# pauxy-qmc/pauxy

Hardware: AMD Instinct MI355X
Metric: walker_steps_per_sec (higher is better)
Workload: dtype f64

## Files before the change

### pauxy_amd/csrc/k_fused.hip

```cpp
#include <cstdlib>
#include <type_traits>

#include "mfma_gemm_wg.h"

#define PF_D 3
#ifndef PF_NW
#define PF_NW 8
#endif
#define PF_NT (64 * PF_NW)
#ifndef PF_LW
#define PF_LW PF_NW
#endif
#define PF_FPW (16 / PF_LW)

#ifdef AFQ_TUNING
#define PF_UNLESS(bits) if (!(a.dbg & (bits)))
#define PF_TUNE(...) __VA_ARGS__
#define PF_STAGE(i) stage_stamp(i)
#define PF_BND(n, i) bnd_stamp(n, i)
#else
#define PF_UNLESS(bits)
#define PF_TUNE(...)
#define PF_STAGE(i)
#define PF_BND(n, i)
#endif

struct PropFusedArgs {
    int M, na, nb, nt, order;
    int t4;
    int dbg;
    unsigned long long *ts;
    int vhs_upper;
    int same_b;
    int b_real;
    int rem4;
    int hyb;
    int symcols;
    int closed_try;
    int contig;
    const cplx *BH1;
    const cplx *vhs;
    cplx *phi;
    const int *alive;
    const void *zero16;
    unsigned long long *n_closed;
};

__device__ inline d2_t lds_read_c(unsigned addr) { return lds_read_b128(addr); }

template <int OFF> __device__ inline d2_t lds_read_off(unsigned addr) {
    d2_t v;
    asm volatile("ds_read_b128 %0, %1 offset:%2" : "=v"(v) : "v"(addr), "n"(OFF));
    return v;
}
__device__ __attribute__((always_inline)) inline d2_t lds_read_frag(unsigned base, int idx) {
    switch (idx) {
    case 0: return lds_read_off<0>(base);
    case 1: return lds_read_off<1024>(base);
    case 2: return lds_read_off<2048>(base);
    case 3: return lds_read_off<3072>(base);
    case 4: return lds_read_off<4096>(base);
    case 5: return lds_read_off<5120>(base);
    case 6: return lds_read_off<6144>(base);
    default: return lds_read_off<7168>(base);
    }
}

template <int OFF> __device__ inline double lds_read_re_off(unsigned addr) {
    double v;
    asm volatile("ds_read_b64 %0, %1 offset:%2" : "=v"(v) : "v"(addr), "n"(OFF));
    return v;
}
__device__ __attribute__((always_inline)) inline double lds_read_frag_re(unsigned base, int idx) {
    switch (idx) {
    case 0: return lds_read_re_off<0>(base);
    case 1: return lds_read_re_off<1024>(base);
    case 2: return lds_read_re_off<2048>(base);
    case 3: return lds_read_re_off<3072>(base);
    case 4: return lds_read_re_off<4096>(base);
    case 5: return lds_read_re_off<5120>(base);
    case 6: return lds_read_re_off<6144>(base);
    default: return lds_read_re_off<7168>(base);
    }
}

__device__ inline void lds_barrier() {
    asm volatile("s_waitcnt lgkmcnt(0)" ::: "memory");
    __builtin_amdgcn_s_barrier();
    asm volatile("" ::: "memory");
}

template <bool NARROW, int FULL>
__global__ __launch_bounds__(PF_NT) void prop_fused_kernel(PropFusedArgs a) {
    extern __shared__ __align__(16) unsigned char smem[];
    const int w = blockIdx.x;
    if (!a.alive[w]) return;
    const int tid = threadIdx.x, lane = tid & 63, wave = __builtin_amdgcn_readfirstlane(tid >> 6);
    const int lr = lane & 15, lk = lane >> 4;
    const int M = a.M, nt = a.nt;
    const int NCH = (M + 7) >> 3;
    const int nrt = (M + 15) >> 4;
    unsigned char *Tf = smem;
    unsigned char *ring = smem + (size_t)NCH * 8192;
    const unsigned tf_l = lds_addr(Tf), ring_l = lds_addr(ring);
    cplx *phi = a.phi + (long)w * M * nt;
    const cplx *vhs = a.vhs + (long)w * M * M;

    PF_TUNE(auto stage_stamp = [&](int i) {
        if (a.ts && w == 0 && wave == 0) {
            unsigned long long t;
            asm volatile("s_memtime %0\n\ts_waitcnt lgkmcnt(0)" : "=s"(t));
            if (lane == 0) a.ts[128 + i] = t;
        }
    };
    auto bnd_stamp = [&](int n, int i) {
        if (a.ts && w == 0 && (wave & 3) == 0 && (n == 3 || n == 4)) {
            unsigned long long t;
            asm volatile("s_memtime %0\n\ts_waitcnt lgkmcnt(0)" : "=s"(t));
            if (lane == 0) a.ts[144 + (wave >> 2) * 8 + (n == 4 ? 4 : 0) + i] = t;
        }
    };)
    PF_STAGE(0);
    const int nob = a.same_b ? 1 : 2;
    const int nphase = 2 * nob + a.order;
    const int G = nphase * NCH;
    const long MM = (long)M * M;
    int gi = 0, gi_phase = 0, gi_c = 0, gi_slot = 0;
    const void *nsrc[PF_FPW];
    bool prepared = false;
    const bool refills = wave >= PF_NW - PF_LW;
    const int lw = wave - (PF_NW - PF_LW);
    const int p_row0 = (lw >> 1) * 16 + lr;
    const int p_kl = 2 * lk + (lw & 1);
    auto prepare = [&]() __attribute__((always_inline)) {
        if (!refills) { prepared = true; return; }
        PF_TUNE(if ((a.dbg & 1024) && gi > 2) { prepared = true; return; })
        const bool in_v = gi_phase >= nob && gi_phase < nob + a.order;
        const int spin = gi_phase < nob ? gi_phase : gi_phase - nob - a.order;
        const cplx *A = in_v ? vhs : a.BH1 + (spin == 1 ? MM : 0L);
        const bool sym_phase = a.vhs_upper && in_v;
        const bool live = gi < G;
        const int k = gi_c * 8 + p_kl;
#pragma unroll
        for (int t = 0; t < PF_FPW; ++t) {
            const int row = p_row0 + t * (PF_LW / 2) * 16;
            const int off = (sym_phase && k < row) ? k * M + row : row * M + k;
            nsrc[t] = (live && row < M && k < M) ? (const void *)(A + off) : a.zero16;
            asm volatile("" : "+v"(nsrc[t]));
        }
        ++gi;
        const bool wrap = gi_c + 1 == NCH;
        gi_c = wrap ? 0 : gi_c + 1;
        gi_phase += wrap ? 1 : 0;
        prepared = true;
    };
    auto issueA = [&]() __attribute__((always_inline)) {
        if (!refills) return;
        if (!prepared) prepare();
        unsigned char *dst = ring + (size_t)gi_slot * 16384;
        PF_TUNE(if (a.dbg & 512) { for (int t = 0; t < PF_FPW; ++t) asm volatile("" ::"v"(nsrc[t]), "s"(dst)); } else)
#pragma unroll
        for (int t = 0; t < PF_FPW; ++t) glds16(nsrc[t], dst + (lw + t * PF_LW) * 1024);
        if (++gi_slot == PF_D) gi_slot = 0;
        prepared = false;
    };
    issueA(); issueA();
    prepare();
    bool closed = false;
    if (a.closed_try) {
        bool same = true;
        for (int p = tid >> 5; p < M; p += PF_NT / 32) {
            const int c = tid & 31;
            if (c < a.na) {
                const cplx x = phi[p * nt + c], y = phi[p * nt + a.na + c];
                same = same && __double_as_longlong(x.x) == __double_as_longlong(y.x) &&
                       __double_as_longlong(x.y) == __double_as_longlong(y.y);
            }
        }
        closed = __builtin_amdgcn_readfirstlane(__syncthreads_and(same ? 1 : 0)) != 0;
        if (closed && tid == 0) atomicAdd(a.n_closed, 1ULL);
    }
    const bool relayout = closed && a.contig;
    const int contig = relayout ? 0 : a.contig, hyb = relayout ? 0 : a.hyb;
    const int sym_n = (a.symcols && !relayout) ? a.na : 0;
    auto wcol = [&](const int c) -> int {
        if (!sym_n) return c;
        if (c < 16) return c;
        if (c < 32) return sym_n + (c - 16);
        if (c < 40) return 16 + (c - 32);
        if (c < 48) return sym_n + 16 + (c - 40);
        const int e = c - 48, extra = sym_n - 24;
        return e < extra ? 24 + e : sym_n + 24 + (e - extra);
    };

    PF_UNLESS((32 | 128))
    for (int e = tid; e < NCH * 512; e += PF_NT) {
        const int j = e & 15, kk = (e >> 4) & 3, pb = (e >> 6) & 1, slot = (e >> 7) & 3, ch = e >> 9;
        const int p = ch * 8 + 2 * kk + pb, sp = contig ? 0 : slot >> 1, col = (contig ? slot : slot & 1) * 16 + j;
        const int ns_ = contig ? nt : sp ? a.nb : a.na, off_ = sp ? a.na : 0;
        const bool ok = p < M && col < ns_;
        const cplx v = phi[ok ? p * nt + off_ + wcol(col) : 0];
        ((d2_t *)Tf)[e] = ok ? (d2_t){v.x, v.y} : (d2_t){0.0, 0.0};
    }
    __syncthreads();

    auto t_ok = [&](int ti, int r) -> bool { return 2 * ti + (r >> 1) < NCH; };
    const unsigned t_lane = (unsigned)((lk & 1) * 1024 + ((lk >> 1) * 16 + lr) * 16);
    auto t_addr = [&](int ti, int r, int cs) -> unsigned {
        unsigned base = t_lane;
        asm volatile("" : "+v"(base));
        return base + (unsigned)(((2 * ti * 4 + cs) * 2) * 1024) + (unsigned)((r >> 1) * 8192 + (r & 1) * 512);
    };

    PF_STAGE(1);
    int ring_slot = 0;
    auto next_chunk = [&]() __attribute__((always_inline)) -> unsigned {
        PF_UNLESS(18)
        asm volatile("s_waitcnt vmcnt(%0)" ::"n"((PF_D - 2) * PF_FPW) : "memory");
        PF_UNLESS(1)
        __builtin_amdgcn_s_barrier();
        PF_UNLESS(2)
        issueA();
        const unsigned sl = ring_l + ring_slot * 16384;
        if (++ring_slot == PF_D) ring_slot = 0;
        return sl;
    };
    auto next_chunk_sync = [&]() __attribute__((always_inline)) -> unsigned {
        asm volatile("s_waitcnt vmcnt(%0)" ::"n"((PF_D - 2) * PF_FPW) : "memory");
        __builtin_amdgcn_s_barrier();
        const unsigned sl = ring_l + ring_slot * 16384;
        ring_slot = ring_slot + 1 == PF_D ? 0 : ring_slot + 1;
        return sl;
    };

    auto one_body = [&](auto nsl_tag, int slot0, bool to_global, auto real_tag, const int rt) __attribute__((always_inline)) {
        constexpr int NSL = decltype(nsl_tag)::value;
        constexpr bool BR = decltype(real_tag)::value;
        constexpr int SS = (NARROW && FULL) ? 2 : 1;
        d4_t P1[NSL], P2[NSL], P3[NSL];
        bool cv[NSL];
#pragma unroll
        for (int j = 0; j < NSL; ++j) {
            P1[j] = (d4_t){0, 0, 0, 0}; P2[j] = (d4_t){0, 0, 0, 0}; P3[j] = (d4_t){0, 0, 0, 0};
            const int cs = slot0 + j * SS;
            cv[j] = rt < nrt && (cs & 1) < ((((cs >> 1) ? a.nb : a.na) + 15) >> 4);
        }
        auto load_frags = [&](unsigned sl, int c, d2_t (&av)[2], d2_t (&bv)[NSL][2]) {
            const unsigned abase = sl + rt * 2048 + lane * 16;
            const unsigned bbase = tf_l + (c * 4 + slot0) * 2048 + lane * 16;
#pragma unroll
            for (int ss = 0; ss < 2; ++ss) {
                if (BR) av[ss][0] = lds_read_frag_re(abase, ss);
                else av[ss] = lds_read_frag(abase, ss);
#pragma unroll
                for (int j = 0; j < NSL; ++j) bv[j][ss] = lds_read_frag(bbase, j * SS * 2 + ss);
            }
        };
        auto mfmas = [&](d2_t (&av)[2], d2_t (&bv)[NSL][2]) {
            __builtin_amdgcn_sched_barrier(0);
            PF_UNLESS(64)
#pragma unroll
            for (int ss = 0; ss < 2; ++ss)
#pragma unroll
                for (int j = 0; j < NSL; ++j)
                    if (FULL || cv[j]) {
                        if (BR) {
                            P1[j] = mfma16(av[ss][0], bv[j][ss][0], P1[j]);
                            P2[j] = mfma16(av[ss][0], bv[j][ss][1], P2[j]);
                        } else {
                            P1[j] = mfma16(av[ss][0], bv[j][ss][0], P1[j]);
                            P2[j] = mfma16(av[ss][1], bv[j][ss][1], P2[j]);
                            P3[j] = mfma16(av[ss][0] + av[ss][1], bv[j][ss][0] + bv[j][ss][1], P3[j]);
                        }
                    }
            __builtin_amdgcn_sched_barrier(0);
            if (!prepared) prepare();
            asm volatile("s_waitcnt lgkmcnt(0)" ::: "memory");
        };
#if PF_NW == 8
        if (FULL) {
            constexpr int NR = 1 + NSL;
            constexpr int RPG = NSL > 1 ? (NR + NSL - 2) / (NSL > 1 ? NSL - 1 : 1) : NR;
            d2_t a0, a1, b0[NSL], b1[NSL];
            auto half = [&](d2_t &ax, d2_t (&bx)[NSL], d2_t &ay, d2_t (&by)[NSL], const unsigned abase, const unsigned bbase,
                            const int ys, const bool fetch, const bool refill) __attribute__((always_inline)) {
                __builtin_amdgcn_sched_barrier(0);
#pragma unroll
                for (int j = 0; j < NSL; ++j) {
                    if (BR) {
                        P1[j] = mfma16(ax[0], bx[j][0], P1[j]);
                        P2[j] = mfma16(ax[0], bx[j][1], P2[j]);
                    } else {
                        P1[j] = mfma16(ax[0], bx[j][0], P1[j]);
                        P2[j] = mfma16(ax[1], bx[j][1], P2[j]);
                        P3[j] = mfma16(ax[0] + ax[1], bx[j][0] + bx[j][1], P3[j]);
                    }
                    __builtin_amdgcn_sched_barrier(0);
                    if (j == 0 && refill) issueA();
                    if (j == 0 && !refill && !prepared) prepare();
                    if (fetch && (j < NSL - 1 || NSL == 1)) {
#pragma unroll
                        for (int q = 0; q < RPG; ++q) {
                            const int r = j * RPG + q;
                            if (r < NR) {
                                if (r == 0) {
                                    if (BR) ay[0] = lds_read_frag_re(abase, ys);
                                    else ay = lds_read_frag(abase, ys);
                                }
                                else by[r - 1] = lds_read_frag(bbase, (r - 1) * SS * 2 + ys);
                            }
                        }
                    }
                    __builtin_amdgcn_sched_barrier(0);
                }
                asm volatile("s_waitcnt lgkmcnt(0)" ::: "memory");
            };
            unsigned sl = next_chunk_sync();
            {
                const unsigned abase = sl + rt * 2048 + lane * 16, bbase = tf_l + slot0 * 2048 + lane * 16;
                if (BR) a0[0] = lds_read_frag_re(abase, 0);
                else a0 = lds_read_frag(abase, 0);
#pragma unroll
                for (int j = 0; j < NSL; ++j) b0[j] = lds_read_frag(bbase, j * SS * 2);
                __builtin_amdgcn_sched_barrier(0);
                issueA();
                asm volatile("s_waitcnt lgkmcnt(0)" ::: "memory");
            }
            for (int c = 0; c < NCH; ++c) {
                const bool more = c + 1 < NCH;
                half(a0, b0, a1, b1, sl + rt * 2048 + lane * 16, tf_l + (c * 4 + slot0) * 2048 + lane * 16, 1, true, false);
                if (more) sl = next_chunk_sync();
                half(a1, b1, a0, b0, sl + rt * 2048 + lane * 16, tf_l + ((c + 1) * 4 + slot0) * 2048 + lane * 16, 0, more, more);
            }
        } else
#endif
        {
#if PF_NW == 16
        d2_t avA[2], bvA[NSL][2];
        for (int c = 0; c < NCH; ++c) {
            load_frags(next_chunk(), c, avA, bvA);
            asm volatile("s_waitcnt lgkmcnt(0)" ::: "memory");
            mfmas(avA, bvA);
        }
#else
        d2_t avA[2], bvA[NSL][2], avB[2], bvB[NSL][2];
        load_frags(next_chunk(), 0, avA, bvA);
        asm volatile("s_waitcnt lgkmcnt(0)" ::: "memory");
        for (int c = 0; c < NCH; c += 2) {
            if (c + 1 < NCH) load_frags(next_chunk(), c + 1, avB, bvB);
            mfmas(avA, bvA);
            if (c + 1 < NCH) {
                if (c + 2 < NCH) load_frags(next_chunk(), c + 2, avA, bvA);
                mfmas(avB, bvB);
            }
        }
#endif
        }
        if (!to_global) __builtin_amdgcn_s_barrier();
        int lk_e = lk, lr_e = lr;
        asm volatile("" : "+v"(lk_e), "+v"(lr_e));
#pragma unroll
        for (int j = 0; j < NSL; ++j)
            if (cv[j]) {
                const int cs = slot0 + j * SS, sp = contig ? 0 : cs >> 1;
                const int ns_ = contig ? nt : sp ? a.nb : a.na, off_ = sp ? a.na : 0;
#pragma unroll
                for (int r = 0; r < 4; ++r) {
                    const double re = BR ? P1[j][r] : P1[j][r] - P2[j][r];
                    const double im = BR ? P2[j][r] : P3[j][r] - P1[j][r] - P2[j][r];
                    if (to_global) {
                        const int row = rt * 16 + lk_e + 4 * r, col = (contig ? cs : cs & 1) * 16 + lr_e;
                        PF_UNLESS(256)
                        if (row < M && col < ns_) phi[(long)row * nt + off_ + wcol(col)] = cmake(re, im);
                    } else if (t_ok(rt, r)) {
                        *(d2_t *)(Tf + t_addr(rt, r, cs)) = (d2_t){re, im};
                    }
                }
            }
    };
    auto one_body_col = [&](bool to_global, auto real_tag, auto rem_tag) __attribute__((always_inline)) {
        constexpr bool BR = decltype(real_tag)::value;
        constexpr bool REM = decltype(rem_tag)::value;
        constexpr int NI = 3;
        constexpr int NG = NI + (REM ? 1 : 0), NR = NI + 1 + (REM ? 1 : 0), RPG = (NR + NG - 2) / (NG - 1);
        const int c0 = wave & 3, r0 = (wave >> 2) * 3;
        const unsigned rem_t = (unsigned)((((12 * 4 + c0) * 2 + ((lane >> 4) & 1)) * 1024) + (((lane >> 5) * 16) + (lane & 15)) * 16);
        const unsigned rem_a = (unsigned)(6 * 2048 + ((lane >> 4) * 16 + (lane & 3)) * 16);
        d4_t P1[NI], P2[NI], P3[NI];
#pragma unroll
        for (int i = 0; i < NI; ++i) { P1[i] = (d4_t){0, 0, 0, 0}; P2[i] = (d4_t){0, 0, 0, 0}; P3[i] = (d4_t){0, 0, 0, 0}; }
        double Q1 = 0.0, Q2 = 0.0, Q3 = 0.0;
        d2_t a0[NI], a1[NI], b0, b1, q0 = (d2_t){0.0, 0.0}, q1 = (d2_t){0.0, 0.0};
        auto half = [&](d2_t (&ax)[NI], d2_t &bx, d2_t &qx, d2_t (&ay)[NI], d2_t &by, d2_t &qy, const unsigned abase,
                        const unsigned bbase, const unsigned qbase, const int ys, const bool fetch, const bool refill)
            __attribute__((always_inline)) {
            __builtin_amdgcn_sched_barrier(0);
#pragma unroll
            for (int gt = 0; gt < NG; ++gt) {
                if (REM && gt == 0) {
                    if (BR) {
                        Q1 = __builtin_amdgcn_mfma_f64_4x4x4f64(qx[0], bx[0], Q1, 0, 0, 0);
                        Q2 = __builtin_amdgcn_mfma_f64_4x4x4f64(qx[0], bx[1], Q2, 0, 0, 0);
                    } else {
                        Q1 = __builtin_amdgcn_mfma_f64_4x4x4f64(qx[0], bx[0], Q1, 0, 0, 0);
                        Q2 = __builtin_amdgcn_mfma_f64_4x4x4f64(qx[1], bx[1], Q2, 0, 0, 0);
                        Q3 = __builtin_amdgcn_mfma_f64_4x4x4f64(qx[0] + qx[1], bx[0] + bx[1], Q3, 0, 0, 0);
                    }
                } else {
                    const int i = REM ? gt - 1 : gt;
                    if (BR) {
                        P1[i] = mfma16(ax[i][0], bx[0], P1[i]);
                        P2[i] = mfma16(ax[i][0], bx[1], P2[i]);
                    } else {
                        P1[i] = mfma16(ax[i][0], bx[0], P1[i]);
                        P2[i] = mfma16(ax[i][1], bx[1], P2[i]);
                        P3[i] = mfma16(ax[i][0] + ax[i][1], bx[0] + bx[1], P3[i]);
                    }
                }
                __builtin_amdgcn_sched_barrier(0);
                if (gt == 0 && refill) issueA();
                if (gt == 0 && !refill && !prepared) prepare();
                if (fetch && gt < NG - 1) {
#pragma unroll
                    for (int q = 0; q < RPG; ++q) {
                        const int r = gt * RPG + q;
                        if (r < NR) {
                            if (r < NI) {
                                if (BR) ay[r][0] = lds_read_frag_re(abase, r * 2 + ys);
                                else ay[r] = lds_read_frag(abase, r * 2 + ys);
                            } else if (r == NI) {
                                by = lds_read_frag(bbase, ys);
                            } else {
                                if (BR) qy[0] = lds_read_frag_re(qbase, ys);
                                else qy = lds_read_frag(qbase, ys);
                            }
                        }
                    }
                }
                __builtin_amdgcn_sched_barrier(0);
            }
            asm volatile("s_waitcnt lgkmcnt(0)" ::: "memory");
        };
        unsigned sl = next_chunk_sync();
        {
            const unsigned abase = sl + r0 * 2048 + lane * 16, bbase = tf_l + c0 * 2048 + lane * 16;
#pragma unroll
            for (int i = 0; i < NI; ++i) {
                if (BR) a0[i][0] = lds_read_frag_re(abase, i * 2);
                else a0[i] = lds_read_frag(abase, i * 2);
            }
            b0 = lds_read_frag(bbase, 0);
            if (REM) {
                if (BR) q0[0] = lds_read_frag_re(sl + rem_a, 0);
                else q0 = lds_read_frag(sl + rem_a, 0);
            }
            __builtin_amdgcn_sched_barrier(0);
            issueA();
            asm volatile("s_waitcnt lgkmcnt(0)" ::: "memory");
        }
        for (int c = 0; c < NCH; ++c) {
            const bool more = c + 1 < NCH;
            half(a0, b0, q0, a1, b1, q1, sl + r0 * 2048 + lane * 16, tf_l + (c * 4 + c0) * 2048 + lane * 16, sl + rem_a, 1, true, false);
            if (more) sl = next_chunk_sync();
            half(a1, b1, q1, a0, b0, q0, sl + r0 * 2048 + lane * 16, tf_l + ((c + 1) * 4 + c0) * 2048 + lane * 16, sl + rem_a, 0, more, more);
        }
        int lk_e = lk, lr_e = lr, ln_e = lane;
        asm volatile("" : "+v"(lk_e), "+v"(lr_e), "+v"(ln_e));
        const int sp = contig ? 0 : c0 >> 1, ns_ = contig ? nt : sp ? a.nb : a.na, off_ = sp ? a.na : 0;
        const int cb = (contig ? c0 : c0 & 1) * 16;
#pragma unroll
        for (int i = 0; i < NI; ++i)
#pragma unroll
            for (int r = 0; r < 4; ++r) {
                const double re = BR ? P1[i][r] : P1[i][r] - P2[i][r];
                const double im = BR ? P2[i][r] : P3[i][r] - P1[i][r] - P2[i][r];
                if (to_global) {
                    const int row = (r0 + i) * 16 + lk_e + 4 * r, col = cb + lr_e;
                    if (row < M && col < ns_) phi[(long)row * nt + off_ + wcol(col)] = cmake(re, im);
                } else if (t_ok(r0 + i, r)) {
                    *(d2_t *)(Tf + t_addr(r0 + i, r, c0)) = (d2_t){re, im};
                }
            }
        if (!to_global) __builtin_amdgcn_s_barrier();
        if (REM) {
            const double re = BR ? Q1 : Q1 - Q2, im = BR ? Q2 : Q3 - Q1 - Q2;
// ... 164 lines not shown
                        }
                        __builtin_amdgcn_sched_barrier(0);
                        if (gt == 0 && refill) issueA();
                        if (gt == 0 && !refill && !prepared) prepare();
                        if (fetch && (gt < NG - 1 || NG == 1)) {
#pragma unroll
                            for (int q = 0; q < RPG; ++q) {
                                const int r = gt * RPG + q;
                                if (r < NR) {
                                    if (r < NI) ay[r] = lds_read_frag(abase, r * 2 + ys);
                                    else if (r < NI + NJ) by[r - NI] = lds_read_frag(bbase, (r - NI) * 2 + ys);
                                    else qy = lds_read_frag(qbase, ys);
                                }
                            }
                        }
                        __builtin_amdgcn_sched_barrier(0);
                    }
                    asm volatile("s_waitcnt lgkmcnt(0)" ::: "memory");
                };
                unsigned sl = next_chunk_sync();
                if (n == 4) PF_BND(4, 0);
                {
                    const unsigned abase = sl + r0 * 2048 + lane * 16, bbase = tf_l + c0 * 2048 + lane * 16;
#pragma unroll
                    for (int i = 0; i < NI; ++i) a0[i] = lds_read_frag(abase, i * 2);
#pragma unroll
                    for (int j = 0; j < NJ; ++j) b0[j] = lds_read_frag(bbase, j * 2);
                    if (REM) q0 = lds_read_frag(sl + rem_a, 0);
                    __builtin_amdgcn_sched_barrier(0);
                    issueA();
                    asm volatile("s_waitcnt lgkmcnt(0)" ::: "memory");
                }
                if (n == 4) PF_BND(4, 1);
                for (int c = 0; c < NCH; ++c) {
                    const bool more = c + 1 < NCH;
                    PF_TUNE(unsigned long long t0, t1, t2, t3; asm volatile("s_memtime %0" : "=s"(t0));)
                    half(a0, b0, q0, a1, b1, q1, sl + r0 * 2048 + lane * 16, tf_l + (c * 4 + c0) * 2048 + lane * 16, sl + rem_a, 1, true, false);
                    PF_TUNE(asm volatile("s_memtime %0" : "=s"(t1));)
                    if (more) sl = next_chunk_sync();
                    PF_TUNE(asm volatile("s_memtime %0" : "=s"(t2));)
                    half(a1, b1, q1, a0, b0, q0, sl + r0 * 2048 + lane * 16, tf_l + ((c + 1) * 4 + c0) * 2048 + lane * 16, sl + rem_a, 0, more, more);
                    PF_TUNE(asm volatile("s_memtime %0\n\ts_waitcnt lgkmcnt(0)" : "=s"(t3));
                            if (a.ts && w == 0 && n == 3 && (wave & 3) == 0 && lane == 0) {
                                unsigned long long *o = a.ts + ((wave >> 2) * 16 + c) * 4;
                                o[0] = t0; o[1] = t1; o[2] = t2; o[3] = t3;
                            }
                            if (a.ts && w == 0 && n == 3 && lane == 0) {
                                unsigned long long *o = a.ts + 256 + (wave * 16 + c) * 4;
                                o[0] = t0; o[1] = t1; o[2] = t2; o[3] = t3;
                            })
                }
            } else
#endif
            {
#if PF_NW == 16
            d2_t avA[NI][2], bvA[NJ][2];
            for (int c = 0; c < NCH; ++c) {
                load_frags(next_chunk(), c, avA, bvA);
                asm volatile("s_waitcnt lgkmcnt(0)" ::: "memory");
                mfmas(avA, bvA);
            }
#else
            d2_t avA[NI][2], bvA[NJ][2], avB[NI][2], bvB[NJ][2];
            if (STAG) {
                auto half = [&](d2_t (&ax)[NI][2], d2_t (&bx)[NJ][2], d2_t (&ay)[NI][2], d2_t (&by)[NJ][2], const int c)
                    __attribute__((always_inline)) {
                    unsigned sl = 0;
                    if (c + 1 < NCH) sl = next_chunk();
                    __builtin_amdgcn_sched_barrier(0);
                    mfma_ss(ax, bx, 1);
                    __builtin_amdgcn_sched_barrier(0);
                    if (!prepared) prepare();
                    if (c + 1 < NCH) {
                        load_frags(sl, c + 1, ay, by);
                        asm volatile("s_waitcnt lgkmcnt(0)" ::: "memory");
                        __builtin_amdgcn_sched_barrier(0);
                        mfma_ss(ay, by, 0);
                        __builtin_amdgcn_sched_barrier(0);
                    }
                };
                load_frags(next_chunk(), 0, avA, bvA);
                asm volatile("s_waitcnt lgkmcnt(0)" ::: "memory");
                __builtin_amdgcn_sched_barrier(0);
                mfma_ss(avA, bvA, 0);
                __builtin_amdgcn_sched_barrier(0);
                for (int c = 0; c < NCH; c += 2) {
                    half(avA, bvA, avB, bvB, c);
                    if (c + 1 < NCH) half(avB, bvB, avA, bvA, c + 1);
                }
            } else {
                load_frags(next_chunk(), 0, avA, bvA);
                asm volatile("s_waitcnt lgkmcnt(0)" ::: "memory");
                for (int c = 0; c < NCH; c += 2) {
                    if (c + 1 < NCH) load_frags(next_chunk(), c + 1, avB, bvB);
                    mfmas(avA, bvA);
                    if (c + 1 < NCH) {
                        if (c + 2 < NCH) load_frags(next_chunk(), c + 2, avA, bvA);
                        mfmas(avB, bvB);
                    }
                }
            }
#endif
            }
            if (n == 3) PF_BND(3, 0);
            const bool store_first = PF_NW == 8 && FULL != 0 && 2 * (r0 + NI) <= NCH - 1;
            if (!store_first) __builtin_amdgcn_s_barrier();
            if (n == 3) PF_BND(3, 1);
            const bool last = n == a.order;
#pragma unroll
            for (int i = 0; i < NI; ++i)
#pragma unroll
                for (int j = 0; j < NJ; ++j)
                    if (FULL || (cv[j] && rv[i])) {
#pragma unroll
                        for (int r = 0; r < 4; ++r) {
                            const double re = (P1[i][j][r] - P2[i][j][r]) * inv_n;
                            const double im = (P3[i][j][r] - P1[i][j][r] - P2[i][j][r]) * inv_n;
                            SR[i][j][r] += re; SI[i][j][r] += im;
                            if (!last && t_ok(r0 + i, r)) *(d2_t *)(Tf + t_addr(r0 + i, r, c0 + j)) = (d2_t){re, im};
                        }
                    }
            if (last) {
#pragma unroll
                for (int i = 0; i < NI; ++i)
#pragma unroll
                    for (int j = 0; j < NJ; ++j)
                        if (FULL || (cv[j] && rv[i])) {
#pragma unroll
                            for (int r = 0; r < 4; ++r)
                                if (t_ok(r0 + i, r))
                                    *(d2_t *)(Tf + t_addr(r0 + i, r, c0 + j)) = (d2_t){SR[i][j][r], SI[i][j][r]};
                        }
            }
            if (store_first) __builtin_amdgcn_s_barrier();
            if (REM) {
                const double re = (Q1 - Q2) * inv_n, im = (Q3 - Q1 - Q2) * inv_n;
                RR += re; RI += im;
                *(d2_t *)(Tf + rem_t) = last ? (d2_t){RR, RI} : (d2_t){re, im};
            }
            if (n == 3) PF_BND(3, 2);
            asm volatile("s_waitcnt lgkmcnt(0)" ::: "memory");
            if (n == 3) PF_BND(3, 3);
            PF_STAGE(2 + n);
        }
    };

    auto taylor_h = [&](auto hf_tag, auto rem_tag, auto nu_tag, const int r0, const int cf, const int cu, const int cr)
        __attribute__((always_inline)) {
        constexpr bool HF = decltype(hf_tag)::value;
        constexpr bool HR = decltype(rem_tag)::value;
        constexpr int NU = decltype(nu_tag)::value;
        constexpr int NI = 2, NRU = HR ? 2 : 0;
        static_assert(FULL == 7, "hybrid tiling: the full wide deal");
        const unsigned u_rd = (unsigned)((lane >> 4) * 256 + (lane & 3) * 16);
        const int ui = lane >> 4, ub = (lane >> 2) & 3;
        const unsigned u_wr = (unsigned)((ub >> 1) * 8192 + (ui & 1) * 1024 + ((2 * (ub & 1) + (ui >> 1)) * 16 + (lane & 3)) * 16);
        auto u_addr = [&](int ti, int u) -> unsigned {
            unsigned base = u_wr;
            asm volatile("" : "+v"(base));
            return base + (unsigned)((2 * ti * 4 + cu) * 2048 + u * 64);
        };
        const unsigned rem_a = (unsigned)(6 * 2048 + ((lane >> 4) * 16 + (lane & 3)) * 16);
        auto rem_t = [&](int t) -> unsigned {
            return (unsigned)((((12 * 4 + cr + t) * 2 + ((lane >> 4) & 1)) * 1024) + (((lane >> 5) * 16) + (lane & 15)) * 16);
        };
        d4_t SR[NI], SI[NI];
        double UR[NI][NU], UI[NI][NU], RR[2] = {0.0, 0.0}, RI[2] = {0.0, 0.0};
#pragma unroll
        for (int i = 0; i < NI; ++i) {
#pragma unroll
            for (int r = 0; r < 4; ++r) {
                d2_t v = (d2_t){0.0, 0.0};
                if (HF) v = *(const d2_t *)(Tf + t_addr(r0 + i, r, cf));
                SR[i][r] = v[0]; SI[i][r] = v[1];
            }
#pragma unroll
            for (int u = 0; u < NU; ++u) { const d2_t v = *(const d2_t *)(Tf + u_addr(r0 + i, u)); UR[i][u] = v[0]; UI[i][u] = v[1]; }
        }
        if (HR) {
#pragma unroll
            for (int t = 0; t < 2; ++t) { const d2_t v = *(const d2_t *)(Tf + rem_t(t)); RR[t] = v[0]; RI[t] = v[1]; }
        }
        struct Frag { d2_t a[NI]; d2_t bf; d2_t bu[NU]; d2_t q; d2_t br[2]; };
        constexpr int NG = NI * NU + NRU + (HF ? NI : 0);
        constexpr int NR = NI + NU + (HF ? 1 : 0) + (HR ? 3 : 0);
        constexpr int NGAP = HF ? NG - 1 : NG - 3;
        constexpr int RPG = (NR + NGAP - 1) / NGAP;
        for (int n = 1; n <= a.order; ++n) {
            double inv_n = 1.0 / n;
            asm volatile("" : "+v"(inv_n));
            d4_t P1[NI], P2[NI], P3[NI];
            double U1[NI][NU], U2[NI][NU], U3[NI][NU], Q1[2] = {0.0, 0.0}, Q2[2] = {0.0, 0.0}, Q3[2] = {0.0, 0.0};
#pragma unroll
            for (int i = 0; i < NI; ++i) {
                P1[i] = (d4_t){0, 0, 0, 0}; P2[i] = (d4_t){0, 0, 0, 0}; P3[i] = (d4_t){0, 0, 0, 0};
#pragma unroll
                for (int u = 0; u < NU; ++u) { U1[i][u] = 0.0; U2[i][u] = 0.0; U3[i][u] = 0.0; }
            }
            auto read_one = [&](Frag &f, const int r, const unsigned sl, const int c, const int ys) __attribute__((always_inline)) {
                const unsigned abase = sl + r0 * 2048 + lane * 16;
                if (r < NI) { f.a[r] = lds_read_frag(abase, r * 2 + ys); return; }
                if (r < NI + NU) {
                    const int u = r - NI;
                    const unsigned ubase = tf_l + (c * 4 + cu) * 2048 + u_rd + ys * 1024;
                    f.bu[u] = u == 0 ? lds_read_off<0>(ubase) : u == 1 ? lds_read_off<64>(ubase) : lds_read_off<128>(ubase);
                    return;
                }
                int k = r - NI - NU;
                if (HF) {
                    if (k == 0) { f.bf = lds_read_frag(tf_l + (c * 4 + cf) * 2048 + lane * 16, ys); return; }
                    --k;
                }
                if (HR) {
                    if (k == 0) f.q = lds_read_frag(sl + rem_a, ys);
                    else f.br[k - 1] = lds_read_frag(tf_l + (c * 4 + cr + k - 1) * 2048 + lane * 16, ys);
                }
            };
            auto half = [&](Frag &x, Frag &y, const unsigned sl, const int c, const int ys, const bool fetch, const bool refill)
                __attribute__((always_inline)) {
                __builtin_amdgcn_sched_barrier(0);
#pragma unroll
                for (int g = 0; g < NG; ++g) {
                    if (g < NI * NU) {
                        const int i = g / NU, u = g % NU;
                        U1[i][u] = __builtin_amdgcn_mfma_f64_4x4x4f64(x.a[i][0], x.bu[u][0], U1[i][u], 0, 0, 0);
                        U2[i][u] = __builtin_amdgcn_mfma_f64_4x4x4f64(x.a[i][1], x.bu[u][1], U2[i][u], 0, 0, 0);
                        U3[i][u] = __builtin_amdgcn_mfma_f64_4x4x4f64(x.a[i][0] + x.a[i][1], x.bu[u][0] + x.bu[u][1], U3[i][u], 0, 0, 0);
                    } else if (g < NI * NU + NRU) {
                        const int t = g - NI * NU;
                        Q1[t] = __builtin_amdgcn_mfma_f64_4x4x4f64(x.q[0], x.br[t][0], Q1[t], 0, 0, 0);
                        Q2[t] = __builtin_amdgcn_mfma_f64_4x4x4f64(x.q[1], x.br[t][1], Q2[t], 0, 0, 0);
                        Q3[t] = __builtin_amdgcn_mfma_f64_4x4x4f64(x.q[0] + x.q[1], x.br[t][0] + x.br[t][1], Q3[t], 0, 0, 0);
                    } else {
                        const int i = g - NI * NU - NRU;
                        P1[i] = mfma16(x.a[i][0], x.bf[0], P1[i]);
                        P2[i] = mfma16(x.a[i][1], x.bf[1], P2[i]);
                        P3[i] = mfma16(x.a[i][0] + x.a[i][1], x.bf[0] + x.bf[1], P3[i]);
                    }
                    __builtin_amdgcn_sched_barrier(0);
                    if (g == 0 && refill) issueA();
                    if (g == 0 && !refill && !prepared) prepare();
                    if (fetch && g < NGAP) {
#pragma unroll
                        for (int q = 0; q < RPG; ++q)
                            if (g * RPG + q < NR) read_one(y, g * RPG + q, sl, c, ys);
                    }
                    __builtin_amdgcn_sched_barrier(0);
                }
                asm volatile("s_waitcnt lgkmcnt(0)" ::: "memory");
            };
            Frag f0, f1;
            f0.q = (d2_t){0.0, 0.0}; f1.q = (d2_t){0.0, 0.0};
            unsigned sl = next_chunk_sync();
#pragma unroll
            for (int r = 0; r < NR; ++r) read_one(f0, r, sl, 0, 0);
            __builtin_amdgcn_sched_barrier(0);
            issueA();
            asm volatile("s_waitcnt lgkmcnt(0)" ::: "memory");
            for (int c = 0; c < NCH; ++c) {
                const bool more = c + 1 < NCH;
                PF_TUNE(unsigned long long t0, t1, t2, t3; asm volatile("s_memtime %0" : "=s"(t0));)
                half(f0, f1, sl, c, 1, true, false);
                PF_TUNE(asm volatile("s_memtime %0" : "=s"(t1));)
                if (more) sl = next_chunk_sync();
                PF_TUNE(asm volatile("s_memtime %0" : "=s"(t2));)
                half(f1, f0, sl, c + 1, 0, more, more);
                PF_TUNE(asm volatile("s_memtime %0\n\ts_waitcnt lgkmcnt(0)" : "=s"(t3));
                        if (a.ts && w == 0 && n == 3 && lane == 0) {
                            unsigned long long *o = a.ts + 256 + (wave * 16 + c) * 4;
                            o[0] = t0; o[1] = t1; o[2] = t2; o[3] = t3;
                        })
            }
            const bool last = n == a.order;
#pragma unroll
            for (int i = 0; i < NI; ++i) {
                if (HF) {
#pragma unroll
                    for (int r = 0; r < 4; ++r) {
                        const double re = (P1[i][r] - P2[i][r]) * inv_n, im = (P3[i][r] - P1[i][r] - P2[i][r]) * inv_n;
                        SR[i][r] += re; SI[i][r] += im;
                        *(d2_t *)(Tf + t_addr(r0 + i, r, cf)) = last ? (d2_t){SR[i][r], SI[i][r]} : (d2_t){re, im};
                    }
                }
#pragma unroll
                for (int u = 0; u < NU; ++u) {
                    const double re = (U1[i][u] - U2[i][u]) * inv_n, im = (U3[i][u] - U1[i][u] - U2[i][u]) * inv_n;
                    UR[i][u] += re; UI[i][u] += im;
                    *(d2_t *)(Tf + u_addr(r0 + i, u)) = last ? (d2_t){UR[i][u], UI[i][u]} : (d2_t){re, im};
                }
            }
            __builtin_amdgcn_s_barrier();
            if (HR) {
#pragma unroll
                for (int t = 0; t < 2; ++t) {
                    const double re = (Q1[t] - Q2[t]) * inv_n, im = (Q3[t] - Q1[t] - Q2[t]) * inv_n;
                    RR[t] += re; RI[t] += im;
                    *(d2_t *)(Tf + rem_t(t)) = last ? (d2_t){RR[t], RI[t]} : (d2_t){re, im};
                }
            }
            asm volatile("s_waitcnt lgkmcnt(0)" ::: "memory");
        }
    };

#ifdef AFQ_TUNING
#include "k_fused_t4.inc"
#endif
    auto mirror_spin = [&]() __attribute__((always_inline)) {
        lds_barrier();
        for (int e = tid; e < NCH * 256; e += PF_NT) {
            const int ch = e >> 8, i = e & 255;
            ((d2_t *)Tf)[ch * 512 + 256 + i] = ((const d2_t *)Tf)[ch * 512 + i];
        }
        asm volatile("s_waitcnt lgkmcnt(0)" ::: "memory");
    };
#if PF_NW == 16
    {
        using I1 = std::integral_constant<int, 1>;
        using I2 = std::integral_constant<int, 2>;
        const int g = wave >> 2;
        if (g & 1) taylor(I2{}, I1{}, std::true_type{}, 2 * g, wave & 3, g == 3 ? 1 : 2, std::false_type{});
        else taylor(I2{}, I1{}, std::false_type{}, 2 * g, wave & 3, 2, std::false_type{});
    }
#else
    PF_TUNE(if (a.t4) taylor4(); else)
    if (NARROW && FULL) {
        using I1 = std::integral_constant<int, 1>;
        using I2 = std::integral_constant<int, 2>;
        if (closed) {
            taylor(I1{}, I1{}, std::false_type{}, wave < 6 ? wave : wave - 6, 0, 1, std::false_type{});
            mirror_spin();
        }
        else if (wave < 4) taylor(I2{}, I1{}, std::false_type{}, 2 * (wave & 1), 2 * (wave >> 1), 2, std::false_type{});
        else taylor(I1{}, I1{}, std::false_type{}, 4 + (wave & 1), 2 * ((wave - 4) >> 1), 1, std::false_type{});
    }
    else if (NARROW) {
        using I1 = std::integral_constant<int, 1>;
        using I2 = std::integral_constant<int, 2>;
        if (wave < 4) taylor(I2{}, I1{}, std::false_type{}, 2 * (wave & 1), 2 * (wave >> 1), 2, std::false_type{});
        else if (nrt <= 6) taylor(I2{}, I1{}, std::true_type{}, 4 + (wave & 1), 2 * ((wave - 4) >> 1), 1, std::false_type{});
        else taylor(I2{}, I1{}, std::true_type{}, (wave & 1) ? 6 : 4, 2 * ((wave - 4) >> 1), (wave & 1) ? 1 : 2, std::false_type{});
    }
    else if (FULL == 7 && contig) {
        if constexpr (FULL == 7) {
            using I1 = std::integral_constant<int, 1>;
            using I2 = std::integral_constant<int, 2>;
            auto deal = [&](auto nu) __attribute__((always_inline)) {
                if (wave == 0 || wave == 2) taylor(I2{}, I2{}, std::false_type{}, wave, 0, 2, std::false_type{});
                else if (wave == 1 || wave == 3) taylor_h(std::true_type{}, std::false_type{}, nu, wave - 1, 2, 3, 0);
                else if (wave == 4 || wave == 6) taylor(I1{}, I1{}, std::true_type{}, 4, (wave - 4) >> 1, 1, std::true_type{});
                else if (wave == 5) taylor(I1{}, I2{}, std::true_type{}, 5, 0, 1, std::false_type{});
                else taylor_h(std::true_type{}, std::true_type{}, nu, 4, 2, 3, 2);
            };
            if (hyb == 2) deal(I2{});
            else deal(I1{});
        }
    }
    else if (FULL == 7 && hyb) {
        if constexpr (FULL == 7) {
            using I1 = std::integral_constant<int, 1>;
            using I2 = std::integral_constant<int, 2>;
            using I3 = std::integral_constant<int, 3>;
            auto deal = [&](auto nu) __attribute__((always_inline)) {
                if (wave < 4) taylor_h(std::true_type{}, std::false_type{}, nu, 2 * (wave >> 1), 2 * (wave & 1), 2 * (wave & 1) + 1, 0);
                else if (wave < 6) taylor(I2{}, I1{}, std::true_type{}, 4, 2 * (wave - 4), 2, std::false_type{});
                else taylor_h(std::false_type{}, std::true_type{}, nu, 4, 0, 2 * (wave - 6) + 1, 2 * (wave - 6));
            };
            if (hyb == 3) deal(I3{});
            else if (hyb == 2) deal(I2{});
            else deal(I1{});
        }
    }
    else if (FULL >= 5 && closed) {
        using I1 = std::integral_constant<int, 1>;
        using I2 = std::integral_constant<int, 2>;
        const int cs = wave & 1;
        if (wave < 4) taylor(I2{}, I1{}, std::false_type{}, 2 * (wave >> 1), cs, 2, std::false_type{});
        else if constexpr (FULL == 7) {
            if (a.rem4) {
                if (wave < 6) taylor(I1{}, I1{}, std::true_type{}, 4, cs, 1, std::true_type{});
                else taylor(I1{}, I1{}, std::true_type{}, 5, cs, 1, std::false_type{});
            } else {
                if (wave < 6) taylor(I2{}, I1{}, std::true_type{}, 4, cs, 2, std::false_type{});
                else taylor(I1{}, I1{}, std::true_type{}, 6, cs, 1, std::false_type{});
            }
        }
        else taylor(I1{}, I1{}, std::true_type{}, (FULL == 6 && wave >= 6) ? 5 : 4, cs, 1, std::false_type{});
        mirror_spin();
    }
    else if (wave < 4) taylor(std::integral_constant<int, 2>{}, std::integral_constant<int, 2>{}, std::false_type{}, 2 * (wave >> 1), 2 * (wave & 1), 2, std::false_type{});
    else if constexpr (FULL == 7) {
        if (a.rem4) taylor(std::integral_constant<int, 2>{}, std::integral_constant<int, 1>{}, std::true_type{}, 4, wave - 4, 2, std::true_type{});
        else taylor(std::integral_constant<int, 3>{}, std::integral_constant<int, 1>{}, std::true_type{}, 4, wave - 4, 3, std::false_type{});
    }
    else if (FULL >= 5) taylor(std::integral_constant<int, FULL >= 5 ? FULL - 4 : 1>{}, std::integral_constant<int, 1>{}, std::true_type{}, 4, wave - 4, FULL - 4, std::false_type{});
    else taylor(std::integral_constant<int, 3>{}, std::integral_constant<int, 1>{}, std::true_type{}, 4, wave - 4, 3, std::false_type{});
#endif
    if (a.order == 0) lds_barrier();

    one_body_stage(true);
    asm volatile("s_waitcnt vmcnt(0)" ::: "memory");
    PF_STAGE(9);
}

int k_prop_fused_supported(afq_handle *h) {
    return !h->no_fused && !h->vhs_diag && h->nv == 1 && h->M <= 104 && h->na <= 32 && h->nb <= 32 && (h->nb > 0 || AFQ_KNOB_SET("AFQ_PF_NB0"));
}

int k_prop_fused(afq_handle *h) {
    PropFusedArgs a;
    a.M = h->M; a.na = h->na; a.nb = h->nb; a.nt = h->nt; a.order = h->exp_order;
    a.vhs_upper = h->vhs_upper ? 1 : 0;
    a.t4 = (h->M <= 100 && AFQ_KNOB_SET("AFQ_T4")) ? 1 : 0;
    a.dbg = AFQ_KNOB_INT("AFQ_PF_DBG", 0);
    a.ts = nullptr;
#ifdef AFQ_TUNING
    static unsigned long long *ts_dev = nullptr;
    static int ts_launch = 0;
    if (AFQ_KNOB_SET("AFQ_PF_TS")) {
        if (!ts_dev) { hipMalloc(&ts_dev, (256 + 512) * 8); hipMemset(ts_dev, 0, (256 + 512) * 8); }
        a.ts = ts_dev;
    }
#endif
    a.same_b = (h->bh1_same && !AFQ_KNOB_SET("AFQ_NO_SAME_B")) ? 1 : 0;
    a.b_real = (h->bh1_real && !AFQ_KNOB_SET("AFQ_NO_REAL_B")) ? 1 : 0;
    a.rem4 = (h->M > 96 && h->M <= 100 && !AFQ_KNOB_SET("AFQ_PF_NOREM")) ? 1 : 0;
    a.hyb = 0;
    if (a.rem4 && h->na > 16 && h->nb > 16 && h->na <= 28 && h->nb <= 28 && (h->na - 13) / 4 == (h->nb - 13) / 4 &&
        PF_NW == 8 && AFQ_KNOB_SET("AFQ_PF_HYB"))
        a.hyb = (h->na - 13) / 4;
    a.contig = 0; a.symcols = 0;
    if (a.rem4 && a.same_b && h->na > 16 && h->nb > 16 && h->nt > 48 && h->nt <= 56 && PF_NW == 8 && !a.hyb &&
        !AFQ_KNOB_SET("AFQ_PF_NOCONTIG")) {
        a.contig = 1;
        a.hyb = (h->nt - 48 + 3) / 4;
    }
    a.symcols = (a.contig && h->na == h->nb && !AFQ_KNOB_SET("AFQ_PF_NOSYM")) ? 1 : 0;
    a.closed_try = 0;
    a.BH1 = h->BH1; a.vhs = h->vhs; a.phi = h->phi; a.alive = h->alive; a.zero16 = h->zero_page;
    a.n_closed = h->counters + 3;
    const int NCH = (h->M + 7) / 8;
    const size_t lds = (size_t)NCH * 8192 + (size_t)PF_D * 16384;
    static size_t lds_set[6][AFQ_MAX_DEVICES] = {{0}, {0}, {0}, {0}, {0}, {0}};
    const bool narrow = h->na <= 16 && h->nb <= 16;
    KernelTrace kt(h, AFQ_K_PROPAGATOR);
    {
        const int nrt_ = (h->M + 15) / 16, ct = (h->na + 15) / 16 + (h->nb + 15) / 16;
        const double ksteps = 2.0 * NCH;
        const double per_pass = ksteps * (2048.0 * (a.rem4 ? nrt_ - 1 : nrt_) * ct + 512.0 * (a.rem4 ? ct : 0));
        const double taylor_pass = a.contig ? ksteps * (2048.0 * (nrt_ - 1) * 3 + 512.0 * (nrt_ - 1) * a.hyb + 512.0 * 4)
                                   : a.hyb ? ksteps * (2048.0 * (nrt_ - 1) * 2 + 512.0 * (nrt_ - 1) * 2 * a.hyb + 512.0 * 4) : per_pass;
        h->issued_flops[AFQ_K_PROPAGATOR] = (3.0 * h->exp_order * taylor_pass + 2.0 * (a.b_real ? 2.0 : 3.0) * per_pass) * h->nw;
        h->prop_issued_open = h->issued_flops[AFQ_K_PROPAGATOR] / h->nw;
        const int cta = (h->na + 15) / 16;
        const double closed_pass = ksteps * (2048.0 * (a.rem4 ? nrt_ - 1 : nrt_) * cta + 512.0 * (a.rem4 ? cta : 0));
        h->prop_issued_closed = 3.0 * h->exp_order * closed_pass + 2.0 * (a.b_real ? 2.0 : 3.0) * per_pass;
    }
    const int nrt = (h->M + 15) / 16;
    const bool nofull = PF_NW != 8 || AFQ_KNOB_SET("AFQ_PF_NOFULL");
    const int full = nofull ? 0 : narrow ? (nrt == 6 ? 6 : 0) : (nrt >= 5 && h->na > 16 && h->nb > 16 ? nrt : 0);
    a.closed_try = (a.same_b && h->na == h->nb && h->exp_order > 0 && full != 0 && PF_NW == 8 && !a.t4 &&
                    (a.contig ? a.symcols != 0 : a.hyb == 0) && !AFQ_KNOB_SET("AFQ_PF_NOCLOSED")) ? 1 : 0;
#define PF_LAUNCH_(NARROW_, FULL_, SLOT_)                                                                     \
    do {                                                                                                      \
        AFQ_HIP(h, afq_raise_lds((const void *)prop_fused_kernel<NARROW_, FULL_>, lds, lds_set[SLOT_]));      \
        AFQ_LAUNCH(h, (prop_fused_kernel<NARROW_, FULL_>), dim3(h->nw), dim3(PF_NT), lds, h->stream, a);      \
    } while (0)
    if (narrow && full) PF_LAUNCH_(true, 6, 0);
    else if (narrow) PF_LAUNCH_(true, 0, 1);
    else if (full == 7) PF_LAUNCH_(false, 7, 2);
    else if (full == 6) PF_LAUNCH_(false, 6, 3);
    else if (full == 5) PF_LAUNCH_(false, 5, 4);
    else PF_LAUNCH_(false, 0, 5);
#undef PF_LAUNCH_
    AFQ_POST(h);
#ifdef AFQ_TUNING
    if (a.ts && ++ts_launch == 30) {
        unsigned long long t[256 + 512];
        hipStreamSynchronize(h->stream);
        hipMemcpy(t, a.ts, sizeof(t), hipMemcpyDeviceToHost);
        fprintf(stderr, "PF_STAGE ticks: phi->T %lld | one-body %lld | Taylor", (long long)(t[129] - t[128]), (long long)(t[130] - t[129]));
        for (int n = 1; n <= h->exp_order && n <= 6; ++n) fprintf(stderr, " %lld", (long long)(t[130 + n] - t[129 + n]));
        for (int wv = 0; wv < 2; ++wv) {
            const unsigned long long *o = t + 144 + wv * 8;
            fprintf(stderr, "\nPF_BND wave %d: loop end -> barrier %lld | epilogue + T writes %lld | barrier %lld | next_chunk %lld | fragment reads %lld",
                    wv * 4, (long long)(o[1] - o[0]), (long long)(o[2] - o[1]), (long long)(o[3] - o[2]), (long long)(o[4] - o[3]), (long long)(o[5] - o[4]));
        }
        fprintf(stderr, "\n");
        fprintf(stderr, " | one-body + store %lld | total %lld\n", (long long)(t[137] - t[130 + h->exp_order]), (long long)(t[137] - t[128]));
        for (int wv = 0; wv < 8; ++wv) {
            const unsigned long long *o = t + 256 + (wv * 16 + 5) * 4, *o0 = t + 256 + 5 * 4, *o6 = t + 256 + (wv * 16 + 6) * 4;
            fprintf(stderr, "PF_ALL wave %d (product 3, chunk 5): start %+5lld  halfA %5lld  sync %5lld (released at %+5lld)  halfB %5lld  | chunk period %lld\n",
                    wv, (long long)(o[0] - o0[0]), (long long)(o[1] - o[0]), (long long)(o[2] - o[1]), (long long)(o[2] - o0[0]),
                    (long long)(o[3] - o[2]), (long long)(o6[0] - o[0]));
        }
        for (int wv = 0; wv < 2; ++wv)
            for (int c = 0; c < (h->M + 7) / 8; ++c) {
                const unsigned long long *o = t + (wv * 16 + c) * 4;
                fprintf(stderr, "PF_TS wave %d chunk %2d: halfA %5lld  sync %5lld  halfB %5lld  | since chunk start of wave 0: %lld\n",
                        wv * 4, c, (long long)(o[1] - o[0]), (long long)(o[2] - o[1]), (long long)(o[3] - o[2]),
                        (long long)(o[0] - t[c * 4]));
            }
    }
#endif
    return AFQ_OK;
}
```

Baseline: 1.037 million.

## Keep V matrix register-resident across Taylor terms in wide full kernel

Adds a VRES kernel variant for the wide 7-row-tile case. Each wave loads its rows of the V matrix into 26 registers once, then reuses them across all Taylor expansion terms, so V no longer streams through the LDS ring on every order. The second spin is handled by swapping the spin halves in LDS and rerunning the pass, or by mirroring when walkers are closed-shell. This raises register pressure and forces the non-contiguous layout, and it only applies when closed_try is set and the exx hint is off.

Measured after the change: 1.049 million (median of 6 runs). 1.2% higher.

```diff
diff --git a/pauxy_amd/csrc/k_fused.hip b/pauxy_amd/csrc/k_fused.hip
--- a/pauxy_amd/csrc/k_fused.hip
+++ b/pauxy_amd/csrc/k_fused.hip
@@ -90,8 +90,9 @@
     asm volatile("" ::: "memory");
 }
 
-template <bool NARROW, int FULL>
+template <bool NARROW, int FULL, bool VRES = false>
 __global__ __launch_bounds__(PF_NT) void prop_fused_kernel(PropFusedArgs a) {
+    static_assert(!VRES || (!NARROW && FULL == 7 && PF_NW == 8), "register-resident V: the wide full deal with 7 row tiles");
     extern __shared__ __align__(16) unsigned char smem[];
     const int w = blockIdx.x;
     if (!a.alive[w]) return;
@@ -122,7 +123,8 @@
     };)
     PF_STAGE(0);
     const int nob = a.same_b ? 1 : 2;
-    const int nphase = 2 * nob + a.order;
+    const int ord_r = VRES ? 0 : a.order;
+    const int nphase = 2 * nob + ord_r;
     const int G = nphase * NCH;
     const long MM = (long)M * M;
     int gi = 0, gi_phase = 0, gi_c = 0, gi_slot = 0;
@@ -135,8 +137,8 @@
     auto prepare = [&]() __attribute__((always_inline)) {
         if (!refills) { prepared = true; return; }
         PF_TUNE(if ((a.dbg & 1024) && gi > 2) { prepared = true; return; })
-        const bool in_v = gi_phase >= nob && gi_phase < nob + a.order;
-        const int spin = gi_phase < nob ? gi_phase : gi_phase - nob - a.order;
+        const bool in_v = gi_phase >= nob && gi_phase < nob + ord_r;
+        const int spin = gi_phase < nob ? gi_phase : gi_phase - nob - ord_r;
         const cplx *A = in_v ? vhs : a.BH1 + (spin == 1 ? MM : 0L);
         const bool sym_phase = a.vhs_upper && in_v;
         const bool live = gi < G;
@@ -163,6 +165,15 @@
         for (int t = 0; t < PF_FPW; ++t) glds16(nsrc[t], dst + (lw + t * PF_LW) * 1024);
         if (++gi_slot == PF_D) gi_slot = 0;
         prepared = false;
+    };
+    constexpr int VK = VRES ? 26 : 1;
+    constexpr int VD = 3;
+    d2_t vs[VK];
+    const int v_row = (VRES && wave == 6 && a.rem4) ? 96 + (lane & 3) : wave * 16 + lr;
+    auto vload = [&](const int idx, const int row) __attribute__((always_inline)) {
+        const int k = (idx >> 1) * 8 + 2 * lk + (idx & 1);
+        const int off = (a.vhs_upper && k < row) ? k * M + row : row * M + k;
+        vs[idx] = *(const d2_t *)((row < M && k < M) ? (const void *)(vhs + off) : a.zero16);
     };
     issueA(); issueA();
     prepare();
@@ -180,7 +191,7 @@
         closed = __builtin_amdgcn_readfirstlane(__syncthreads_and(same ? 1 : 0)) != 0;
         if (closed && tid == 0) atomicAdd(a.n_closed, 1ULL);
     }
-    const bool relayout = closed && a.contig;
+    const bool relayout = (VRES || closed) && a.contig;
     const int contig = relayout ? 0 : a.contig, hyb = relayout ? 0 : a.hyb;
     const int sym_n = (a.symcols && !relayout) ? a.na : 0;
     auto wcol = [&](const int c) -> int {
@@ -951,6 +962,117 @@
         }
     };
 
+    auto taylor_v = [&](auto role_tag, auto fill_tag, const int c0) __attribute__((always_inline)) {
+        constexpr int ROLE = decltype(role_tag)::value;
+        constexpr bool FILL = decltype(fill_tag)::value;
+        constexpr int NCV = VK / 2;
+        const int r0 = wave;
+        int vrow = v_row;
+        asm volatile("" : "+v"(vrow));
+        auto rem_t = [&](int cs) -> unsigned {
+            return (unsigned)((((12 * 4 + cs) * 2 + ((lane >> 4) & 1)) * 1024) + (((lane >> 5) * 16) + (lane & 15)) * 16);
+        };
+        d4_t SR[2], SI[2];
+        double RR[2] = {0.0, 0.0}, RI[2] = {0.0, 0.0};
+#pragma unroll
+        for (int j = 0; j < 2; ++j) {
+#pragma unroll
+            for (int r = 0; r < 4; ++r) {
+                d2_t v = (d2_t){0.0, 0.0};
+                if (ROLE == 0 && t_ok(r0, r)) v = *(const d2_t *)(Tf + t_addr(r0, r, c0 + j));
+                SR[j][r] = v[0]; SI[j][r] = v[1];
+            }
+            if (ROLE == 1) { const d2_t v = *(const d2_t *)(Tf + rem_t(c0 + j)); RR[j] = v[0]; RI[j] = v[1]; }
+        }
+        const unsigned b_lane = tf_l + (unsigned)(c0 * 2048 + lane * 16);
+        auto read_b = [&](d2_t (&b)[2], const int s) __attribute__((always_inline)) {
+            unsigned base = b_lane;
+            asm volatile("" : "+v"(base));
+            base += (unsigned)((s >> 1) * 8192);
+            b[0] = lds_read_frag(base, s & 1);
+            b[1] = lds_read_frag(base, 2 + (s & 1));
+        };
+        auto product = [&](auto fill_now, const int n) __attribute__((always_inline)) {
+            constexpr bool LOAD = decltype(fill_now)::value;
+            const bool last = n == a.order;
+            double inv_n = 1.0 / n;
+            asm volatile("" : "+v"(inv_n));
+            if (!LOAD) {
+#pragma unroll
+                for (int i = 0; i < VK; ++i) asm volatile("" : "+v"(vs[i]));
+            }
+            d4_t P1[2], P2[2], P3[2];
+            double Q1[2] = {0.0, 0.0}, Q2[2] = {0.0, 0.0}, Q3[2] = {0.0, 0.0};
+#pragma unroll
+            for (int j = 0; j < 2; ++j) { P1[j] = (d4_t){0, 0, 0, 0}; P2[j] = (d4_t){0, 0, 0, 0}; P3[j] = (d4_t){0, 0, 0, 0}; }
+            if (ROLE != 2) {
+                auto group = [&](const int j, const d2_t av, const d2_t bj) __attribute__((always_inline)) {
+                    if (ROLE == 0) {
+                        P1[j] = mfma16(av[0], bj[0], P1[j]);
+                        P2[j] = mfma16(av[1], bj[1], P2[j]);
+                        P3[j] = mfma16(av[0] + av[1], bj[0] + bj[1], P3[j]);
+                        asm volatile("" ::"v"(P1[j][0]), "v"(P2[j][0]), "v"(P3[j][0]));
+                    } else {
+                        Q1[j] = __builtin_amdgcn_mfma_f64_4x4x4f64(av[0], bj[0], Q1[j], 0, 0, 0);
+                        Q2[j] = __builtin_amdgcn_mfma_f64_4x4x4f64(av[1], bj[1], Q2[j], 0, 0, 0);
+                        Q3[j] = __builtin_amdgcn_mfma_f64_4x4x4f64(av[0] + av[1], bj[0] + bj[1], Q3[j], 0, 0, 0);
+                        asm volatile("" ::"v"(Q1[j]), "v"(Q2[j]), "v"(Q3[j]));
+                    }
+                };
+                auto kstep = [&](const int s, d2_t (&bx)[2], d2_t (&by)[2]) __attribute__((always_inline)) {
+                    __builtin_amdgcn_sched_barrier(0);
+                    group(0, vs[s], bx[0]);
+                    __builtin_amdgcn_sched_barrier(0);
+                    if (s + 1 < VK) read_b(by, s + 1);
+                    if (LOAD && (s & 1) == 0 && (s >> 1) + VD < NCV) { vload(s + 2 * VD, vrow); vload(s + 2 * VD + 1, vrow); }
+                    __builtin_amdgcn_sched_barrier(0);
+                    group(1, vs[s], bx[1]);
+                    __builtin_amdgcn_sched_barrier(0);
+                    asm volatile("s_waitcnt lgkmcnt(0)" ::: "memory");
+                };
+                d2_t b0[2], b1[2];
+                read_b(b0, 0);
+                asm volatile("s_waitcnt lgkmcnt(0)" ::: "memory");
+#pragma unroll
+                for (int s = 0; s < VK; s += 2) {
+                    kstep(s, b0, b1);
+                    kstep(s + 1, b1, b0);
+                }
+            }
+            lds_barrier();
+            if (ROLE == 0) {
+#pragma unroll
+                for (int j = 0; j < 2; ++j)
+#pragma unroll
+                    for (int r = 0; r < 4; ++r) {
+                        const double re = (P1[j][r] - P2[j][r]) * inv_n;
+                        const double im = (P3[j][r] - P1[j][r] - P2[j][r]) * inv_n;
+                        SR[j][r] += re; SI[j][r] += im;
+                        if (t_ok(r0, r)) *(d2_t *)(Tf + t_addr(r0, r, c0 + j)) = last ? (d2_t){SR[j][r], SI[j][r]} : (d2_t){re, im};
+                    }
+            } else if (ROLE == 1) {
+#pragma unroll
+                for (int j = 0; j < 2; ++j) {
+                    const double re = (Q1[j] - Q2[j]) * inv_n, im = (Q3[j] - Q1[j] - Q2[j]) * inv_n;
+                    RR[j] += re; RI[j] += im;
+                    *(d2_t *)(Tf + rem_t(c0 + j)) = last ? (d2_t){RR[j], RI[j]} : (d2_t){re, im};
+                }
+            }
+            lds_barrier();
+            PF_STAGE(2 + n);
+        };
+        int n = 1;
+        if (FILL) {
+            if (ROLE != 2) {
+#pragma unroll
+                for (int i = 0; i < 2 * VD; ++i) vload(i, vrow);
+            }
+            product(std::true_type{}, 1);
+            n = 2;
+        }
+        for (; n <= a.order; ++n) product(std::false_type{}, n);
+    };
+
 #ifdef AFQ_TUNING
 #include "k_fused_t4.inc"
 #endif
@@ -971,6 +1093,30 @@
         else taylor(I2{}, I1{}, std::false_type{}, 2 * g, wave & 3, 2, std::false_type{});
     }
 #else
+    if constexpr (VRES) {
+        auto swap_spins = [&]() __attribute__((always_inline)) {
+            lds_barrier();
+            for (int e = tid; e < NCH * 256; e += PF_NT) {
+                d2_t *t = (d2_t *)Tf + (e >> 8) * 512 + (e & 255);
+                const d2_t x = t[0], y = t[256];
+                t[0] = y; t[256] = x;
+            }
+            lds_barrier();
+        };
+        auto pass = [&]() __attribute__((always_inline)) {
+            if (wave < 6 || (wave == 6 && !a.rem4)) taylor_v(std::integral_constant<int, 0>{}, std::true_type{}, 0);
+            else if (wave == 6) taylor_v(std::integral_constant<int, 1>{}, std::true_type{}, 0);
+            else taylor_v(std::integral_constant<int, 2>{}, std::true_type{}, 0);
+        };
+        pass();
+        if (closed) {
+            mirror_spin();
+        } else {
+            swap_spins();
+            pass();
+            swap_spins();
+        }
+    } else {
     PF_TUNE(if (a.t4) taylor4(); else)
     if (NARROW && FULL) {
         using I1 = std::integral_constant<int, 1>;
@@ -1043,6 +1189,7 @@
     }
     else if (FULL >= 5) taylor(std::integral_constant<int, FULL >= 5 ? FULL - 4 : 1>{}, std::integral_constant<int, 1>{}, std::true_type{}, 4, wave - 4, FULL - 4, std::false_type{});
     else taylor(std::integral_constant<int, 3>{}, std::integral_constant<int, 1>{}, std::true_type{}, 4, wave - 4, 3, std::false_type{});
+    }
 #endif
     if (a.order == 0) lds_barrier();
 
@@ -1089,7 +1236,7 @@
     a.n_closed = h->counters + 3;
     const int NCH = (h->M + 7) / 8;
     const size_t lds = (size_t)NCH * 8192 + (size_t)PF_D * 16384;
-    static size_t lds_set[6][AFQ_MAX_DEVICES] = {{0}, {0}, {0}, {0}, {0}, {0}};
+    static size_t lds_set[7][AFQ_MAX_DEVICES] = {{0}, {0}, {0}, {0}, {0}, {0}, {0}};
     const bool narrow = h->na <= 16 && h->nb <= 16;
     KernelTrace kt(h, AFQ_K_PROPAGATOR);
     {
@@ -1109,17 +1256,25 @@
     const int full = nofull ? 0 : narrow ? (nrt == 6 ? 6 : 0) : (nrt >= 5 && h->na > 16 && h->nb > 16 ? nrt : 0);
     a.closed_try = (a.same_b && h->na == h->nb && h->exp_order > 0 && full != 0 && PF_NW == 8 && !a.t4 &&
                     (a.contig ? a.symcols != 0 : a.hyb == 0) && !AFQ_KNOB_SET("AFQ_PF_NOCLOSED")) ? 1 : 0;
-#define PF_LAUNCH_(NARROW_, FULL_, SLOT_)                                                                     \
+    const bool vres = a.closed_try && full == 7 && !h->exx_open_hint && !AFQ_KNOB_SET("AFQ_PF_NOVRES");
+    if (vres) {
+        const int nrt_ = (h->M + 15) / 16, cta = (h->na + 15) / 16;
+        const double closed_pass = 2.0 * NCH * (2048.0 * (a.rem4 ? nrt_ - 1 : nrt_) * cta + 512.0 * (a.rem4 ? cta : 0));
+        h->prop_issued_open = h->prop_issued_closed + 3.0 * h->exp_order * closed_pass;
+        h->issued_flops[AFQ_K_PROPAGATOR] = h->prop_issued_open * h->nw;
+    }
+#define PF_LAUNCH_(SLOT_, ...)                                                                                \
     do {                                                                                                      \
-        AFQ_HIP(h, afq_raise_lds((const void *)prop_fused_kernel<NARROW_, FULL_>, lds, lds_set[SLOT_]));      \
-        AFQ_LAUNCH(h, (prop_fused_kernel<NARROW_, FULL_>), dim3(h->nw), dim3(PF_NT), lds, h->stream, a);      \
+        AFQ_HIP(h, afq_raise_lds((const void *)prop_fused_kernel<__VA_ARGS__>, lds, lds_set[SLOT_]));         \
+        AFQ_LAUNCH(h, (prop_fused_kernel<__VA_ARGS__>), dim3(h->nw), dim3(PF_NT), lds, h->stream, a);         \
     } while (0)
-    if (narrow && full) PF_LAUNCH_(true, 6, 0);
-    else if (narrow) PF_LAUNCH_(true, 0, 1);
-    else if (full == 7) PF_LAUNCH_(false, 7, 2);
-    else if (full == 6) PF_LAUNCH_(false, 6, 3);
-    else if (full == 5) PF_LAUNCH_(false, 5, 4);
-    else PF_LAUNCH_(false, 0, 5);
+    if (narrow && full) PF_LAUNCH_(0, true, 6);
+    else if (narrow) PF_LAUNCH_(1, true, 0);
+    else if (vres) PF_LAUNCH_(6, false, 7, true);
+    else if (full == 7) PF_LAUNCH_(2, false, 7);
+    else if (full == 6) PF_LAUNCH_(3, false, 6);
+    else if (full == 5) PF_LAUNCH_(4, false, 5);
+    else PF_LAUNCH_(5, false, 0);
 #undef PF_LAUNCH_
     AFQ_POST(h);
 #ifdef AFQ_TUNING
```
